# Fedomn/sqlrs

Hardware: AMD Instinct MI355X
Metric: Mrows/sec for filter->hash-join->group-by pipeline; achieved HBM GB/s vs peak (higher is better)
Workload: dtype int64 keys / f64 sum; 1 GPU; C5 filter(val>0.5) -> hash-join(fact x dim on int64 key) -> group-by(key) COUNT,SUM(f64); fact_rows=1000000000, dim_rows=10000000, groups=10000000, parallelism=single GPU

## Files before the change

sqlrs_amd/csrc/radix_part.hip:

```cpp
#include <cstdio>
#include <cstdlib>

#include "device_utils.hpp"
#include "radix_part.hpp"
#include "radix_part_kernels.hpp"

namespace sq {

namespace {

struct Level {
  std::vector<int64_t> seg_mat, seg_start;
  std::vector<uint32_t> seg_tiles, seg_tile_base;
  int64_t mat_entries = 0;
  uint32_t num_tiles = 0, nseg = 0;
  std::vector<uint8_t> blob;
  BufP dev, tiles;
  const int64_t *d_seg_start = nullptr, *d_seg_mat = nullptr;
  const uint32_t *d_seg_tiles = nullptr, *d_seg_tile_base = nullptr;
};

Level plan_level(const std::vector<int64_t> &seg_start, uint32_t digits, int RP_TILE) {
  Level L;
  L.seg_start = seg_start;
// ... 106 lines not shown
  };
  auto publish = [&](const Cols &c) {
    out->key = c.k; out->v0 = c.v0; out->v1 = c.v1; out->idx = c.idx; out->flags = c.fl; out->rec = c.rec;
  };
  struct SlimLaunch {
    SlimIn in;
    SlimOut out;
    uint32_t kshift, rbits;
    BufP total;
  };
  auto exec_level = [&](int level, uint32_t digits, const Level &L, const RpIn &rin, const RpOut &rout, int64_t sink,
                        BufP *offs_out, BufP premat = nullptr, SlimLaunch *slim = nullptr,
                        const std::function<void(const BufP &)> *before_scatter = nullptr) {
    const int64_t entries = std::max<int64_t>(L.mat_entries, 1);
    BufP mat = premat ? premat : ctx->alloc(4 * (size_t)entries);
    BufP offs = ctx->alloc(4 * (size_t)entries);
    BufP total = ctx->alloc(8);
    if (slim) slim->total = total;
    unsigned nt = L.num_tiles;
    const Tile *tp = (const Tile *)L.tiles->p;
    if (nt && !premat) {
      ProfScope ps(ctx, in.build_side ? "rp_hist_build" : "rp_hist");
#define SQ_RH1(R, PL) rp_hist_kernel<512, R, PL><<<dim3(nt), dim3(512), 0, ctx->stream>>>(rin.key, rin.key_validity, rin.flags, tp, P, p2_bits, level, digits, mat->as<uint32_t>(), kp)
#define SQ_RH(R) do { if (!rin.key_validity && !rin.flags) SQ_RH1(R, true); else SQ_RH1(R, false); } while (0)
      if (ROWS == 12) SQ_RH(12); else SQ_RH(8);
#undef SQ_RH
#undef SQ_RH1
      SQ_HIP(hipGetLastError());
    }
    BufP mat_dm = ctx->alloc(4 * (size_t)entries);
    BufP offs_tm = ctx->alloc(4 * (size_t)entries);
    const size_t tlds = (size_t)RP_TB * (digits + 1) * 4;
    const unsigned tblocks = (unsigned)ceil_div(nt, RP_TB);
    if (nt)
      rp_transpose_kernel<false><<<dim3(tblocks), dim3(256), tlds, ctx->stream>>>(
          mat->as<uint32_t>(), mat_dm->as<uint32_t>(), tp, nt, digits);
    exclusive_scan_u32(ctx, mat_dm->as<uint32_t>(), L.mat_entries, nullptr, offs->as<uint32_t>(),
                       total->as<uint64_t>());
    if (nt)
      rp_transpose_kernel<true><<<dim3(tblocks), dim3(256), tlds, ctx->stream>>>(
          offs->as<uint32_t>(), offs_tm->as<uint32_t>(), tp, nt, digits);
    SQ_HIP(hipGetLastError());
    if (before_scatter) (*before_scatter)(offs);
    if (nt) {
      ProfScope ps(ctx, in.build_side ? "rp_scatter_build" : "rp_scatter");
      uint32_t wgs = std::min<uint32_t>(nt, (uint32_t)ctx->num_cus);
      uint32_t tpw = (uint32_t)ceil_div(nt, wgs);
      wgs = (uint32_t)ceil_div(nt, tpw);
      dim3 g(wgs), b((unsigned)WG);
      const int mode = level == 1 ? (flags ? RP_L1_NULL : RP_L1) : (flags ? RP_LN_FLAG : RP_LN);
      if (slim) {
        const size_t slds = (size_t)RP_TILE * 13 + 1024 + (size_t)WG * 16 + 512 + 128;
        allow_big_lds(ctx, rp_scatter_slim_kernel);
        rp_scatter_slim_kernel<<<g, b, slds, ctx->stream>>>(slim->in, slim->out, tp, p2_bits, digits, offs_tm->as<uint32_t>(), nt, tpw, sink,
                                                           slim->kshift, slim->rbits);
        SQ_HIP(hipGetLastError());
        slim->total = total;
        *offs_out = offs;
        return;
      }
#define SQ_RP1(NV, R, M, PK)                                                                                  \
  do {                                                                                                        \
    constexpr bool can_rec = NV == 1 && PK;                                                                   \
    auto kfn = rp_scatter_kernel<NV, 512, R, M, PK>;                                                          \
    if (can_rec && rout.rec) kfn = rp_scatter_kernel<NV, 512, R, M, PK, can_rec>;                             \
    allow_big_lds(ctx, kfn);                                                                                  \
    kfn<<<g, b, lds, ctx->stream>>>(rin, rout, tp, P, p2_bits, level, digits, offs_tm->as<uint32_t>(), nt, tpw, \
                                    sink, kp);                                                                  \
  } while (0)
#define SQ_RP(NV, R)                                                                                          \
  do {                                                                                                        \
    if (mode == RP_L1) { if (pack) SQ_RP1(NV, R, RP_L1, true); else SQ_RP1(NV, R, RP_L1, false); }            \
    else if (mode == RP_L1_NULL) SQ_RP1(NV, R, RP_L1_NULL, false);                                            \
    else if (mode == RP_LN) { if (pack) SQ_RP1(NV, R, RP_LN, true); else SQ_RP1(NV, R, RP_LN, false); }       \
    else SQ_RP1(NV, R, RP_LN_FLAG, false);                                                                    \
  } while (0)
      if (nv == 2) SQ_RP(2, 8);
      else if (nv == 0) SQ_RP(0, 12); else SQ_RP(1, 12);
#undef SQ_RP1
#undef SQ_RP
      SQ_HIP(hipGetLastError());
    }
    *offs_out = offs;
  };

  auto run_level = [&](int level, uint32_t digits, const std::vector<int64_t> &seg_start, const RpIn &rin,
                       const RpOut &rout, BufP *offs_out, Level *L) {
    *L = plan_level(seg_start, digits, RP_TILE);
    L->tiles = ctx->alloc(sizeof(Tile) * (size_t)std::max<uint32_t>(L->num_tiles, 1));
    upload_level(ctx, *L);
    rp_make_tiles_kernel<<<dim3((unsigned)L->seg_tiles.size()), dim3(256), 0, ctx->stream>>>(
        L->d_seg_start, L->d_seg_mat, L->d_seg_tiles, L->d_seg_tile_base, RP_TILE, (Tile *)L->tiles->p);
    SQ_HIP(hipGetLastError());
    exec_level(level, digits, *L, rin, rout, n, offs_out);
  };

  auto bucket_starts = [&](const Level &L, const BufP &offs, uint32_t digits, int64_t rows,
                           std::vector<uint32_t> *host) -> BufP {
    uint32_t nseg = L.nseg;
    int64_t total = (int64_t)nseg * digits + 1;
    BufP bs = ctx->alloc(4 * (size_t)total);
    rp_bucket_starts_kernel<<<dim3((unsigned)ceil_div(total, 256)), dim3(256), 0, ctx->stream>>>(
        offs->as<uint32_t>(), L.d_seg_mat, L.d_seg_tiles, L.d_seg_start, digits, nseg, rows, bs->as<uint32_t>());
    SQ_HIP(hipGetLastError());
    if (4 * (size_t)total <= ctx->pinned_bytes) {
      const uint32_t *h = (const uint32_t *)ctx->fetch(bs->p, 4 * (size_t)total);
      host->assign(h, h + total);
// ... 79 lines not shown
        csl.log_b = log_b;
        csl.tile = (uint32_t)RP_TILE;
        csl.on = true;
      } else if (use_rec) cc.rec = ctx->alloc(16 * (size_t)pool_rows);
      else {
        cc.k = ctx->alloc(8 * (size_t)pool_rows);
        cc.v0 = nv >= 1 ? ctx->alloc(8 * (size_t)pool_rows) : nullptr;
      }
      ClaimOut co;
      co.key = cc.k ? cc.k->as<uint64_t>() : nullptr;
      co.v0 = cc.v0 ? cc.v0->as<uint64_t>() : nullptr;
      co.rec = cc.rec ? (u64x2 *)cc.rec->p : nullptr;
      co.cursor = cursor;
      co.rend = rend;
      co.kept = (unsigned long long *)cst;
      co.flag = (unsigned int *)(cst + 1);
      co.B = B;
      const int psrc = !in.filter.col ? -1 : ((nv >= 1 && (const void *)in.filter.col == in.vals[0]) ? 1 : 3);
      const size_t clds = (size_t)RP_TILE * 8 * (1 + nv) + (size_t)WG * (4 + 4 + 8 + 8);
      {
        ProfScope ps(ctx, in.filter.col ? "rp_claim_scatter_filter" : "rp_claim_scatter");
        const uint64_t *k = in.keys, *a0 = (const uint64_t *)in.vals[0];
        const int64_t sink = (int64_t)slots_max;
#define SQ_CL1(NV, PS, RC)                                                                                          \
  do {                                                                                                              \
    auto kfn = rp_claim_scatter_kernel<NV, 512, 12, PS, RC>;                                                        \
    allow_big_lds(ctx, kfn);                                                                                        \
    kfn<<<dim3(wgs), dim3(512), clds, ctx->stream>>>(k, a0, in.filter, n, co, P, tiles1c, tpw, sink, kp);           \
  } while (0)
#define SQ_CL(NV, RC)                                                                                               \
  do {                                                                                                              \
    if (psrc < 0) SQ_CL1(NV, -1, RC);                                                                               \
    else if (psrc == 1 && NV >= 1) SQ_CL1(NV, (NV >= 1 ? 1 : 3), RC);                                               \
    else SQ_CL1(NV, 3, RC);                                                                                         \
  } while (0)
        if (claim_slim) {
          SlimClaimOut so;
          so.rows = csl.rows;
          so.cursor = cursor;
          so.rend = rend;
          so.blk_bt = csl.blk_bt->as<uint32_t>();
          so.flag = co.flag;
          so.kept = co.kept;
          so.B = B;
          so.log_b = csl.log_b;
          const char *sd_e = hook("SQLRS_RP_SLIM_DELTA");
          so.max_delta = sd_e ? (uint32_t)std::max(1, std::min(std::atoi(sd_e), 127)) : 127u;
          const size_t slds = (size_t)RP_TILE * (8 + 4 + 2) + (size_t)WG * (4 + 4 + 8 + 8 + 4);
          const size_t slds768 = (size_t)RP_TILE * (8 + 4 + 2) + (size_t)768 * (4 + 4 + 8 + 8 + 4);
#define SQ_CS(W, R, PS, LDS)                                                                                        \
  do {                                                                                                              \
    auto kfn = rp_claim_scatter_slim_kernel<W, R, PS>;                                                              \
    allow_big_lds(ctx, kfn);                                                                                        \
    kfn<<<dim3(wgs), dim3(W), LDS, ctx->stream>>>(k, a0, in.filter, n, so, P, tiles1c, tpw, sink, kp);              \
  } while (0)
          if (psrc < 0) SQ_CS(768, 8, -1, slds768);
          else if (psrc == 1) SQ_CS(768, 8, 1, slds768);
          else SQ_CS(512, 12, 3, slds);
#undef SQ_CS
        } else if (nv == 0) SQ_CL(0, false);
        else if (use_rec) SQ_CL(1, true);
        else SQ_CL(1, false);
#undef SQ_CL
#undef SQ_CL1
        SQ_HIP(hipGetLastError());
      }
      const uint32_t *hp = (const uint32_t *)ctx->fetch(plan->p, plan_bytes);
      uint64_t hc[2];
      std::memcpy(hc, hp + plan_words, 16);
      if (!(uint32_t)hc[1]) {
        out->n = (int64_t)hc[0];
        out->P = P;
        publish(cc);
        if (claim_slim) out->slim = csl;
        out->bstart = plan;
        out->bstart_host.assign(hp, hp + P);
        out->bstart_host.push_back((uint32_t)slots_max);
        out->bend_host.assign(hp + 2 * (size_t)P, hp + 3 * (size_t)P);
        return true;
      }
    }
  }
  if (in.filter.col && p2_bits == 0) return false;

  static const int chunk_env = [] {
    const char *e = hook("SQLRS_RP_CHUNKED");
    return e ? std::atoi(e) : -1;
  }();
  const uint32_t tiles1 = (uint32_t)ceil_div(n, RP_TILE);
  uint32_t cwgs = std::min<uint32_t>(tiles1, (uint32_t)ctx->num_cus);
  if (const char *wg_e = hook("SQLRS_RP_CHUNK_WGS"))
    cwgs = std::max(1u, std::min<uint32_t>(cwgs, (uint32_t)std::atoi(wg_e)));
  const uint32_t ctpw = (uint32_t)ceil_div(tiles1, std::max(cwgs, 1u));
  cwgs = (uint32_t)ceil_div(tiles1, std::max(ctpw, 1u));
  const uint64_t spare_chunks = (uint64_t)cwgs * (d1 + 1);
  const uint64_t CAP = (uint64_t)RP_TILE;
  bool chunked = p2_bits != 0 && !flags && chunk_env != 0 && d1 <= (uint32_t)WG &&
                 (chunk_env == 1 || spare_chunks * CAP <= (uint64_t)n);
  if (in.filter.col && !chunked) return false;
  if (chunked) {
    const char *slim_e = hook("SQLRS_RP_SLIM");
    const bool slim_on = pack && kp.dense && nv == 1 && (size_t)P * 4 <= 24 * 1024 &&
                         kp.rbits + SLIM_LOCAL_BITS + 7 <= 32 && kp.rbits + p2_bits + SLIM_LOCAL_BITS <= 32 &&
                         !(slim_e && std::atoi(slim_e) == 0) && !(hook("SQLRS_RP_H2") && std::atoi(hook("SQLRS_RP_H2")) == 0);
    const char *sd_e = hook("SQLRS_RP_SLIM_DELTA");
    const uint32_t slim_delta = sd_e ? (uint32_t)std::max(1, std::min<int>(std::atoi(sd_e), (int)SLIM_RUNS - 1)) : SLIM_RUNS - 1;
    const uint64_t arena = (uint64_t)ctpw + d1 + 1 +
                           (slim_on ? (uint64_t)d1 * (uint64_t)ceil_div((int64_t)ctpw, (int64_t)slim_delta + 1) : 0);
    const uint64_t max_chunks = arena * cwgs;
    if (max_chunks * (CAP + RP_CHUNK_SKEW) + WG * (uint64_t)cwgs > 0xffffffffull) {
      if (in.filter.col) return false;
      chunked = false;
    }
    if (chunked && slim_on) {
      const size_t pool_rows = (size_t)max_chunks * (CAP + RP_CHUNK_SKEW) + (size_t)1024 * cwgs;
      const uint32_t digits2 = 1u << p2_bits;
      auto slim_alloc = [&](size_t rows, BufP &b0, BufP &b1) {
        SlimRowsView v;
        b0 = ctx->alloc(8 * rows);
        b1 = ctx->alloc(4 * rows);
        v.v = b0->as<uint64_t>();
        v.w = b1->as<uint32_t>();
        return v;
      };
      BufP cb0, cb1;
      BufP clen = ctx->alloc_zero(4 * (size_t)max_chunks);
      BufP cdig = ctx->alloc(4 * (size_t)max_chunks), cbase = ctx->alloc(4 * (size_t)max_chunks);
      BufP cstart = ctx->alloc(2 * (size_t)max_chunks * SLIM_RUNS);
      SQ_HIP(hipMemsetAsync(cstart->p, 0xff, 2 * (size_t)max_chunks * SLIM_RUNS, ctx->stream));
      BufP ctr = ctx->alloc_zero(8);
      BufP chist = ctx->alloc(4 * (size_t)max_chunks * digits2);
      SlimChunkOut so;
      so.rows = slim_alloc(pool_rows, cb0, cb1);
      so.chunk_len = clen->as<uint32_t>();
      so.chunk_dig = cdig->as<uint32_t>();
      so.chunk_base = cbase->as<uint32_t>();
      so.cstart = cstart->as<uint16_t>();
      so.counter = ctr->as<unsigned int>();
      so.max_chunks = (uint32_t)max_chunks;
      so.cap = (uint32_t)CAP;
      so.arena = (uint32_t)arena;
      so.hist = chist->as<uint32_t>();
      so.kshift = kp.rbits + p2_bits;
      so.max_delta = slim_delta;
      {
        const char *cc_e = hook("SQLRS_RP_CONC");
        so.conc_eighths = cc_e ? (uint32_t)std::max(1, std::min(std::atoi(cc_e), 9)) : 3u;
      }
      const int psrc = !in.filter.col ? -1 : ((const void *)in.filter.col == in.vals[0] ? 1 : 3);
      const size_t clds = (size_t)RP_TILE * 14 + (size_t)WG * (4 + 4 + 8 + 8 + 4 + 4) + (size_t)P * 4;
      {
        ProfScope ps(ctx, in.filter.col ? "rp_chunk_scatter_filter" : "rp_chunk_scatter");
        const int64_t sink = (int64_t)max_chunks * (CAP + RP_CHUNK_SKEW);
        const size_t clds768 = (size_t)RP_TILE * 14 + (size_t)768 * (4 + 4 + 8 + 8 + 4 + 4) + (size_t)P * 4;
#define SQ_SL(W, R, PS, LDS)                                                                                        \
  do {                                                                                                              \
    auto kfn = rp_chunk_scatter_slim_kernel<W, R, PS>;                                                              \
    allow_big_lds(ctx, kfn);                                                                                        \
    kfn<<<dim3(cwgs), dim3(W), LDS, ctx->stream>>>(in.keys, (const uint64_t *)in.vals[0], in.filter, n, so, P, p2_bits, d1, \
                                                   tiles1, ctpw, sink, kp);                                         \
  } while (0)
        if (psrc < 0) SQ_SL(768, 8, -1, clds768); else if (psrc == 1) SQ_SL(768, 8, 1, clds768); else SQ_SL(512, 12, 3, clds);
#undef SQ_SL
        SQ_HIP(hipGetLastError());
      }
      Level L2;
      L2.nseg = d1;
      const LevelLayout lay(d1);
      L2.dev = ctx->alloc(lay.total);
      bind_level(L2, lay);
      L2.tiles = ctx->alloc(sizeof(Tile) * (size_t)max_chunks);
      BufP totals = ctx->alloc(24);
      BufP tile_chunk = ctx->alloc(4 * (size_t)max_chunks);
      BufP plan = ctx->alloc(sizeof(ChunkPlan));
      SQ_HIP(hipMemsetAsync(plan->p, 0, sizeof(ChunkPlan), ctx->stream));
      const unsigned pblocks = (unsigned)std::min<uint64_t>(ceil_div((int64_t)max_chunks, 256 * 8), 128);
      rp_chunk_count_kernel<<<dim3(pblocks), dim3(256), 0, ctx->stream>>>(so.chunk_len, so.chunk_dig, so.counter, so.max_chunks,
                                                                        so.max_chunks, (uint32_t)RP_TILE, plan->as<ChunkPlan>());
      rp_chunk_prefix_kernel<<<dim3(1), dim3(64), 0, ctx->stream>>>(
          plan->as<ChunkPlan>(), so.counter, d1, digits2, (int64_t *)L2.d_seg_start, (int64_t *)L2.d_seg_mat,
          (uint32_t *)L2.d_seg_tiles, (uint32_t *)L2.d_seg_tile_base, totals->as<uint64_t>());
      rp_chunk_assign_kernel<<<dim3(pblocks), dim3(256), 0, ctx->stream>>>(
          so.chunk_len, so.chunk_dig, so.counter, so.max_chunks, so.max_chunks, digits2, (uint32_t)CAP, (uint32_t)RP_TILE,
          L2.d_seg_tiles, L2.d_seg_tile_base, plan->as<ChunkPlan>(), (Tile *)L2.tiles->p, tile_chunk->as<uint32_t>());
      SQ_HIP(hipGetLastError());
      const uint64_t *ht = (const uint64_t *)ctx->fetch(totals->p, 24);
      const uint64_t ntiles = ht[0], kept = ht[1], overflow = ht[2];
      if (overflow) return false;
      L2.num_tiles = (uint32_t)ntiles;
      L2.mat_entries = (int64_t)ntiles * digits2;
      out->n = (int64_t)kept;
      out->P = P;
      if (kept == 0) {
        out->bstart_host.assign((size_t)P + 1, 0u);
        out->bstart = nullptr;
        return true;
      }
      const size_t np = (size_t)kept + 1024;
      PartitionedRows::Slim &sl = out->slim;
      sl = PartitionedRows::Slim();
      sl.rows = slim_alloc(np, sl.buf0, sl.buf1);
      SlimLaunch sln;
      sln.in.rows = so.rows;
      sln.in.tile_chunk = tile_chunk->as<uint32_t>();
      sln.in.cstart = so.cstart;
      sln.out.rows = sl.rows;
      sln.kshift = so.kshift;
      sln.rbits = kp.rbits;
      BufP offs2;
      BufP premat = ctx->alloc(4 * (size_t)L2.mat_entries);
      rp_hist_from_chunks_kernel<<<dim3((unsigned)ceil_div(L2.mat_entries, 256)), dim3(256), 0, ctx->stream>>>(
          so.hist, tile_chunk->as<uint32_t>(), L2.mat_entries, digits2, premat->as<uint32_t>());
      SQ_HIP(hipGetLastError());
// ... 198 lines not shown
```

sqlrs_amd/csrc/radix_part_kernels.hpp:

```cpp
#pragma once
#include "device_utils.hpp"
#include "radix_part.hpp"

#ifdef RP_NT_STORES
#define RP_ST(ptr, val) __builtin_nontemporal_store((val), (ptr))
#else
#define RP_ST(ptr, val) (*(ptr) = (val))
#endif

namespace sq {


constexpr int vmcnt_imm(int n) { return (n & 0xF) | ((n >> 4) << 14) | 0x0F70; }

struct Tile {
  int64_t start;
  uint32_t len;
  uint32_t stride;
  int64_t mat;
};

__device__ __forceinline__ uint32_t xcd_tile(uint32_t b, uint32_t nb) {
  uint32_t q = nb >> 3, r = nb & 7, x = b & 7, i = b >> 3;
  return x * q + min(x, r) + i;
// ... 433 lines not shown
        if ((uint32_t)(j * RP_WG) < staged_len) store_row(j, staged_len);
        rank_row(j, len);
      }
#ifndef RP_PREFETCH_LATE
      __builtin_amdgcn_s_waitcnt(0x0F70);
#else
      rp_chunk_load<NV, RP_WG, RP_ROWS, PSRC>(key, v0, v1, flt.col, nstart, nlen, nxt);
      __builtin_amdgcn_s_waitcnt(vmcnt_imm(NLOADS < 63 ? NLOADS : 63));
#endif
      __syncthreads();
      scan_and_stage();
      staged_len = s_total;
      cur = nxt;
      len = nlen;
      cur_start = nstart;
    }
#pragma unroll
    for (int j = 0; j < RP_ROWS; j++)
      if ((uint32_t)(j * RP_WG) < staged_len) store_row(j, staged_len);
  }
  if (owner) {
    out.chunk_len[cur_id] = cfill;
    out.chunk_dig[cur_id] = threadIdx.x;
  }
  if (H2) {
    __syncthreads();
    close_id[threadIdx.x] = owner ? cur_id : 0xffffffffu;
    __syncthreads();
    flush_closed();
  }
}

constexpr uint32_t SLIM_RUNS = 128;
constexpr uint32_t SLIM_LOCAL_BITS = 13;
struct SlimChunkOut {
  SlimRowsView rows;
  uint32_t *chunk_len;
  uint32_t *chunk_dig;
  uint32_t *chunk_base;
  uint16_t *cstart;
  unsigned int *counter;
  uint32_t max_chunks, cap, arena;
  uint32_t *hist;
  uint32_t kshift;
  uint32_t max_delta;
  uint32_t conc_eighths;
};

template <int RP_ROWS> struct SlimCur {
  uint32_t off[RP_ROWS];
  uint64_t a0[RP_ROWS];
};

template <int RP_WG, int RP_ROWS, int PSRC>
__global__ __launch_bounds__(RP_WG, 1) void rp_chunk_scatter_slim_kernel(
    const uint64_t *__restrict__ key, const uint64_t *__restrict__ v0, RowFilter flt, int64_t n, SlimChunkOut out,
    uint32_t P, uint32_t p2_bits, uint32_t digits, uint32_t num_tiles, uint32_t tiles_per_wg, int64_t sink, KeyPack kp) {
  constexpr uint32_t RP_TILE = RP_WG * RP_ROWS;
  static_assert(RP_TILE <= (1u << SLIM_LOCAL_BITS), "row inside a tile must fit SLIM_LOCAL_BITS");
  extern __shared__ __attribute__((aligned(16))) unsigned char smem[];
  uint64_t *sv0 = (uint64_t *)smem;
  uint32_t *sw = (uint32_t *)(sv0 + RP_TILE);
  uint16_t *sdig = (uint16_t *)(sw + RP_TILE);
  uint32_t *cnt = (uint32_t *)(sdig + RP_TILE);
  uint32_t *split = cnt + RP_WG;
  int64_t *gb0 = (int64_t *)(split + RP_WG);
  int64_t *gb1 = gb0 + RP_WG;
  uint32_t *room_s = (uint32_t *)(gb1 + RP_WG);
  uint32_t *close_id = room_s + RP_WG;
  uint32_t *h2 = close_id + RP_WG;
  __shared__ uint32_t s_wsum[RP_WG / 64];
  __shared__ uint32_t s_total;
  __shared__ uint32_t s_next;
  const uint32_t d2n = 1u << p2_bits;
  const uint32_t inmask = (1u << out.kshift) - 1u;

  const uint32_t t0 = blockIdx.x * tiles_per_wg;
  const uint32_t t1 = min(num_tiles, t0 + tiles_per_wg);
  uint32_t cur_id = blockIdx.x * out.arena + min(threadIdx.x, digits - 1), cfill = 0, cbase = 0;
  bool opened = false;
  if (threadIdx.x == 0) s_next = digits;
  const bool owner = threadIdx.x < digits;
  room_s[threadIdx.x] = out.cap;
  for (uint32_t i = threadIdx.x; i < digits * d2n; i += RP_WG) h2[i] = 0;
  auto tile_start = [&](uint32_t t) { return (int64_t)t * RP_TILE; };
  auto tile_len = [&](uint32_t t) { return (uint32_t)min((int64_t)RP_TILE, n - (int64_t)t * RP_TILE); };

  ChunkRegs<1, RP_ROWS, PSRC> nxt;
  SlimCur<RP_ROWS> cur;
  uint32_t dr[RP_ROWS];
  uint32_t cur_tile = 0;
  auto take_rows = [&](uint32_t len, uint32_t nxt_tile, bool report) {
#pragma unroll
    for (int j = 0; j < RP_ROWS; j++) {
      bool keep = (uint32_t)(j * RP_WG) + threadIdx.x < len;
      if (PSRC == 1) keep = keep && row_passes(flt, nxt.a0[j]);
      if (PSRC == 3) keep = keep && row_passes(flt, nxt.pv[PSRC == 3 ? j : 0]);
      const uint64_t off = nxt.k[j] - kp.kmin;
      if (keep && off > kp.range) {
        if (kp.oob && report) key_out_of_range(kp, (uint32_t)((int64_t)nxt_tile * RP_TILE + (uint32_t)(j * RP_WG) + threadIdx.x));
        keep = false;
      }
      cur.off[j] = keep ? (uint32_t)off : 0xffffffffu;
      cur.a0[j] = nxt.a0[j];
    }
  };
  __shared__ uint32_t s_conc;
  uint32_t conc_digit = 0xffffffffu;
  uint32_t w_b0 = 0xffffffffu, w_base = 0;
  auto plan_wave = [&]() {
    w_b0 = 0xffffffffu;
    if (conc_digit == 0xffffffffu) return;
#pragma unroll
    for (int j = 0; j < RP_ROWS; j++) {
      const uint32_t bkt = cur.off[j] >> kp.rbits;
      const uint64_t m = __ballot(cur.off[j] != 0xffffffffu && (bkt >> p2_bits) == conc_digit);
      if (w_b0 == 0xffffffffu && m) w_b0 = (uint32_t)__builtin_amdgcn_readlane((int)bkt, __builtin_ctzll(m));
    }
    if (w_b0 == 0xffffffffu) return;
    uint32_t total = 0;
#pragma unroll
    for (int j = 0; j < RP_ROWS; j++)
      total += (uint32_t)__popcll(__ballot(cur.off[j] != 0xffffffffu && (cur.off[j] >> kp.rbits) == w_b0));
    if (total < 4u * RP_ROWS) {
      w_b0 = 0xffffffffu;
      return;
    }
    const uint32_t d0 = w_b0 >> p2_bits;
    uint32_t base = 0;
    if (lane_id() == 0) base = atomicAdd(&cnt[d0], total);
    w_base = (uint32_t)__builtin_amdgcn_readfirstlane((int)base);
    const uint32_t room = room_s[d0];
    const uint32_t nlo = room > w_base ? min(room - w_base, total) : 0u;
    if (lane_id() == 0) atomicAdd(&h2[w_b0], nlo + ((total - nlo) << 16));
  };
  auto rank_row = [&](int j) {
    dr[j] = 0xffffffffu;
    const bool in = cur.off[j] != 0xffffffffu;
    const uint32_t bkt = cur.off[j] >> kp.rbits;
    if (w_b0 != 0xffffffffu) {
      const bool peer = in && bkt == w_b0;
      const uint64_t same = __ballot(peer);
      if (peer) dr[j] = ((w_b0 >> p2_bits) << 16) | (w_base + (uint32_t)mbcnt(same));
      w_base += (uint32_t)__popcll(same);
      if (in && !peer) {
        const uint32_t d = bkt >> p2_bits;
        const uint32_t r = atomicAdd(&cnt[d], 1u);
        atomicAdd(&h2[bkt], r < room_s[d] ? 1u : 0x10000u);
        dr[j] = (d << 16) | r;
      }
      return;
    }
    if (in) {
      const uint32_t d = bkt >> p2_bits;
      const uint32_t r = atomicAdd(&cnt[d], 1u);
      atomicAdd(&h2[bkt], r < room_s[d] ? 1u : 0x10000u);
      dr[j] = (d << 16) | r;
    }
  };
  auto flush_closed = [&]() {
    for (uint32_t i = threadIdx.x; i < digits * d2n; i += RP_WG) {
      const uint32_t c = close_id[i >> p2_bits];
      if (c == 0xffffffffu) continue;
      const uint32_t v = h2[i];
      out.hist[(size_t)c * d2n + (i & (d2n - 1))] = v & 0xffffu;
      h2[i] = v >> 16;
    }
  };
  auto take_chunk = [&]() {
    const uint32_t o = atomicAdd(&s_next, 1u);
    if (o >= out.arena) out.counter[1] = 1;
    return blockIdx.x * out.arena + min(o, out.arena - 1);
  };
  auto scan_and_stage = [&]() {
    const uint32_t c = cnt[threadIdx.x];
    if (c * 8u >= (uint32_t)RP_TILE * out.conc_eighths) s_conc = threadIdx.x + 1;
    const uint32_t inc = wave_iscan_u32(c);
    if (lane_id() == 63) s_wsum[wave_id()] = inc;
    __syncthreads();
    conc_digit = s_conc - 1u;
    uint32_t wbase = 0, tot = 0;
    for (int w = 0; w < RP_WG / 64; w++) {
      if (w < wave_id()) wbase += s_wsum[w];
      tot += s_wsum[w];
    }
    const uint32_t ls = wbase + inc - c;
    if (threadIdx.x == 0) s_total = tot;
    const uint32_t room = min(c, out.cap - cfill);
    int64_t g0 = (int64_t)cur_id * (out.cap + RP_CHUNK_SKEW) + cfill, g1 = 0;
    uint32_t closing = 0xffffffffu;
    if (owner && c > 0) {
      if (!opened) {
        opened = true;
        cbase = cur_tile;
        out.chunk_base[cur_id] = cur_tile;
      }
      out.cstart[(size_t)cur_id * SLIM_RUNS + (cur_tile - cbase)] = (uint16_t)cfill;
    }
    if (owner && c > room) {
      out.chunk_len[cur_id] = out.cap;
      out.chunk_dig[cur_id] = threadIdx.x;
      closing = cur_id;
      cur_id = take_chunk();
      cfill = c - room;
      cbase = cur_tile;
      out.chunk_base[cur_id] = cur_tile;
      out.cstart[(size_t)cur_id * SLIM_RUNS] = 0;
      g1 = (int64_t)cur_id * (out.cap + RP_CHUNK_SKEW);
    } else {
      cfill += c;
      if (owner && opened && cur_tile + 1 - cbase > out.max_delta) {
        out.chunk_len[cur_id] = cfill;
        out.chunk_dig[cur_id] = threadIdx.x;
        closing = cur_id;
        cur_id = take_chunk();
        cfill = 0;
        opened = false;
      }
    }
    close_id[threadIdx.x] = closing;
    cnt[threadIdx.x] = ls;
    split[threadIdx.x] = ls + room;
    gb0[threadIdx.x] = g0 - (int64_t)ls;
    gb1[threadIdx.x] = g1 - (int64_t)(ls + room);
    room_s[threadIdx.x] = out.cap - cfill;
    __syncthreads();
    flush_closed();
#pragma unroll
    for (int j = 0; j < RP_ROWS; j++) {
      if (dr[j] == 0xffffffffu) continue;
      const uint32_t d = dr[j] >> 16;
      const uint32_t p = cnt[d] + (dr[j] & 0xffffu);
      const uint32_t local = (uint32_t)(j * RP_WG) + threadIdx.x;
      sv0[p] = cur.a0[j];
      sw[p] = (cur.off[j] & inmask) | (local << out.kshift);
      sdig[p] = (uint16_t)d;
    }
    __syncthreads();
  };
  auto store_row = [&](int j, uint32_t len) {
    const uint32_t p = j * RP_WG + threadIdx.x;
    const uint32_t d = min((uint32_t)sdig[p], (uint32_t)(RP_WG - 1));
    int64_t g = (p < split[d] ? gb0[d] : gb1[d]) + p;
    if (p >= len) g = sink + (int64_t)blockIdx.x * RP_WG + threadIdx.x;
    slim_store(out.rows, g, sw[p], sv0[p]);
  };

  if (t0 < t1) {
    uint32_t len = tile_len(t0);
    cur_tile = t0;
    rp_chunk_load<1, RP_WG, RP_ROWS, PSRC>(key, v0, nullptr, flt.col, tile_start(t0), len, nxt);
    __builtin_amdgcn_s_waitcnt(0x0F70);
    take_rows(len, t0, true);
    cnt[threadIdx.x] = 0;
    if (threadIdx.x == 0) s_conc = 0;
    __syncthreads();
    plan_wave();
#pragma unroll
    for (int j = 0; j < RP_ROWS; j++) rank_row(j);
    __syncthreads();
    scan_and_stage();
    uint32_t staged_len = s_total;
    uint32_t tcur = min(t0 + 1, t1 - 1);
    len = tile_len(tcur);
    cur_tile = tcur;
    rp_chunk_load<1, RP_WG, RP_ROWS, PSRC>(key, v0, nullptr, flt.col, tile_start(tcur), len, nxt);
    __builtin_amdgcn_s_waitcnt(0x0F70);
    take_rows(len, tcur, tcur != t0);
    for (uint32_t ti = t0 + 1; ti < t1; ti++) {
      const uint32_t tnext = min(ti + 1, t1 - 1);
      const uint32_t nlen = tile_len(tnext);
      rp_chunk_load<1, RP_WG, RP_ROWS, PSRC>(key, v0, nullptr, flt.col, tile_start(tnext), nlen, nxt);
      cnt[threadIdx.x] = 0;
      if (threadIdx.x == 0) s_conc = 0;
      __syncthreads();
      plan_wave();
#pragma unroll
      for (int j = 0; j < RP_ROWS; j++) {
        if ((uint32_t)(j * RP_WG) < staged_len) store_row(j, staged_len);
        rank_row(j);
      }
      __builtin_amdgcn_s_waitcnt(0x0F70);
      __syncthreads();
      scan_and_stage();
      staged_len = s_total;
      take_rows(nlen, tnext, tnext != ti);
      cur_tile = tnext;
    }
#pragma unroll
    for (int j = 0; j < RP_ROWS; j++)
      if ((uint32_t)(j * RP_WG) < staged_len) store_row(j, staged_len);
  }
  if (owner) {
    out.chunk_len[cur_id] = cfill;
    out.chunk_dig[cur_id] = threadIdx.x;
  }
  __syncthreads();
  close_id[threadIdx.x] = owner ? cur_id : 0xffffffffu;
  __syncthreads();
  flush_closed();
}

struct SlimIn {
  SlimRowsView rows;
  const uint32_t *tile_chunk;
  const uint16_t *cstart;
};
struct SlimOut {
  SlimRowsView rows;
};
template <int RP_ROWS> struct SlimRegs {
  uint64_t a0[RP_ROWS];
  uint32_t w[RP_ROWS];
  uint32_t goff;
  uint16_t cs0, cs1;
};
template <int RP_WG, int RP_ROWS>
__device__ __forceinline__ void rp_slim_load(const SlimIn &in, const Tile &t, uint32_t tile_index,
                                             const uint32_t *__restrict__ offs, uint32_t digits, SlimRegs<RP_ROWS> &r) {
#pragma unroll
  for (int j = 0; j < RP_ROWS; j++) {
    const int64_t row = t.start + min((uint32_t)(j * RP_WG) + threadIdx.x, t.len - 1);
    slim_load_nt(in.rows, row, r.w[j], r.a0[j]);
  }
  r.goff = offs[(int64_t)tile_index * digits + min(threadIdx.x, digits - 1)];
  const uint16_t *cs = in.cstart + (size_t)in.tile_chunk[tile_index] * SLIM_RUNS;
  r.cs0 = cs[lane_id()];
  r.cs1 = cs[64 + lane_id()];
}

__global__ __launch_bounds__(512, 1) void rp_scatter_slim_kernel(SlimIn in, SlimOut out, const Tile *__restrict__ tiles,
                                                                uint32_t p2_bits, uint32_t digits,
                                                                const uint32_t *__restrict__ offs, uint32_t num_tiles,
                                                                uint32_t tiles_per_wg, int64_t sink, uint32_t kshift,
                                                                uint32_t rbits) {
  constexpr int RP_WG = 512, RP_ROWS = 12, RP_TILE = RP_WG * RP_ROWS;
  static_assert(SLIM_RUNS == 128 && RP_TILE / 64 <= 128, "one mask word per 64 positions of a chunk");
  extern __shared__ __attribute__((aligned(16))) unsigned char smem[];
  uint64_t *sv0 = (uint64_t *)smem;
  unsigned long long *rmask = (unsigned long long *)(sv0 + RP_TILE);
  int64_t *gbase = (int64_t *)(rmask + 128);
  uint32_t *sw = (uint32_t *)(gbase + RP_WG);
  uint32_t *cnt = sw + RP_TILE;
  uint32_t *lstart = cnt + RP_WG;
  uint32_t *rpre = lstart + RP_WG;
  uint8_t *sdig = (uint8_t *)(rpre + 128);
  uint8_t *rdelta = sdig + RP_TILE;
  __shared__ uint32_t s_wsum[RP_WG / 64];
  __shared__ uint32_t s_psum;
  const uint32_t d2mask = (1u << p2_bits) - 1u, slotmask = (1u << rbits) - 1u;
  const uint64_t le_mask = (2ull << lane_id()) - 1ull;

  const uint32_t t0 = blockIdx.x * tiles_per_wg;
  const uint32_t t1 = min(num_tiles, t0 + tiles_per_wg);
  if (t0 >= t1) return;
  auto tile_of = [&](uint32_t slot) { return slot; };
  SlimRegs<RP_ROWS> cur, nxt;
  uint32_t dr[RP_ROWS];
  __shared__ uint32_t s_conc;
  bool conc_hint = false;
  auto rank_row = [&](int j, uint32_t len) {
    dr[j] = 0xffffffffu;
    const bool in = (uint32_t)(j * RP_WG) + threadIdx.x < len;
    const uint32_t d = (cur.w[j] >> rbits) & d2mask;
    if (conc_hint) {
      const uint64_t m = __ballot(in);
      if (m) {
        const int first = __builtin_ctzll(m);
        const uint32_t d0 = (uint32_t)__builtin_amdgcn_readlane((int)d, first);
        const bool peer = in && d == d0;
        const uint64_t same = __ballot(peer);
        if (__popcll(same) >= 8) {
          uint32_t base = 0;
          if ((int)lane_id() == first) base = atomicAdd(&cnt[d0], (uint32_t)__popcll(same));
          base = (uint32_t)__builtin_amdgcn_readlane((int)base, first);
          if (peer) dr[j] = (d0 << 16) | (base + (uint32_t)mbcnt(same));
          else if (in) dr[j] = (d << 16) | atomicAdd(&cnt[d], 1u);
          return;
        }
      }
    }
    if (in) dr[j] = (d << 16) | atomicAdd(&cnt[d], 1u);
  };
  auto build_runs = [&](uint32_t len) {
    if (wave_id() != 0) return;
    const bool f0 = cur.cs0 < len, f1 = cur.cs1 < len;
    const uint64_t b0 = __ballot(f0), b1 = __ballot(f1);
    const uint64_t lt = le_mask >> 1;
    if (f0) {
      rdelta[__popcll(b0 & lt)] = (uint8_t)lane_id();
      atomicOr(&rmask[cur.cs0 >> 6], 1ull << (cur.cs0 & 63));
    }
    if (f1) {
      rdelta[__popcll(b0) + __popcll(b1 & lt)] = (uint8_t)(64 + lane_id());
      atomicOr(&rmask[cur.cs1 >> 6], 1ull << (cur.cs1 & 63));
    }
  };
  auto scan_and_stage = [&](uint32_t tile_len) {
    uint32_t c = cnt[threadIdx.x];
    if (tile_len && c * 10u >= tile_len * 9u) s_conc = 1;
    uint32_t inc = wave_iscan_u32(c);
    if (lane_id() == 63) s_wsum[wave_id()] = inc;
    uint32_t pc = 0, pinc = 0;
    if (threadIdx.x < 128) {
      pc = (uint32_t)__popcll(rmask[threadIdx.x]);
      pinc = wave_iscan_u32(pc);
      if (threadIdx.x == 63) s_psum = pinc;
    }
    __syncthreads();
    conc_hint = s_conc != 0;
    uint32_t wbase = 0;
    for (int w = 0; w < wave_id(); w++) wbase += s_wsum[w];
    uint32_t ls = wbase + inc - c;
    lstart[threadIdx.x] = ls;
    gbase[threadIdx.x] = (int64_t)cur.goff - (int64_t)ls;
    if (threadIdx.x < 128) rpre[threadIdx.x] = pinc - pc + (threadIdx.x >= 64 ? s_psum : 0u);
    __syncthreads();
#pragma unroll
    for (int j = 0; j < RP_ROWS; j++) {
      if (dr[j] == 0xffffffffu) continue;
      const uint32_t p = lstart[dr[j] >> 16] + (dr[j] & 0xffffu);
      const uint32_t g = (uint32_t)(j * (RP_WG / 64)) + (uint32_t)wave_id();
      const uint32_t k = rpre[g] + (uint32_t)__popcll(rmask[g] & le_mask) - 1u;
      const uint32_t delta = rdelta[k & (SLIM_RUNS - 1)];
      const uint32_t w = cur.w[j];
      sv0[p] = cur.a0[j];
      sw[p] = (w & slotmask) | (((w >> kshift) & ((1u << SLIM_LOCAL_BITS) - 1u)) << rbits) | (delta << (rbits + SLIM_LOCAL_BITS));
      sdig[p] = (uint8_t)(dr[j] >> 16);
    }
    __syncthreads();
  };
  auto store_row = [&](int j, uint32_t len) {
    const uint32_t p = j * RP_WG + threadIdx.x;
    int64_t g = gbase[sdig[p] & d2mask] + p;
    if (p >= len) g = sink + threadIdx.x;
    slim_store(out.rows, g, sw[p], sv0[p]);
  };

  uint32_t tix = tile_of(t0);
  Tile t = tiles[tix];
  rp_slim_load<RP_WG, RP_ROWS>(in, t, tix, offs, digits, cur);
  __builtin_amdgcn_s_waitcnt(0x0F70);
  cnt[threadIdx.x] = 0;
  if (threadIdx.x < 128) rmask[threadIdx.x] = 0;
  if (threadIdx.x == 0) s_conc = 0;
  __syncthreads();
#pragma unroll
  for (int j = 0; j < RP_ROWS; j++) rank_row(j, t.len);
  build_runs(t.len);
  __syncthreads();
  scan_and_stage(t.len);
  uint32_t staged_len = t.len;
  tix = tile_of(min(t0 + 1, t1 - 1));
  t = tiles[tix];
  rp_slim_load<RP_WG, RP_ROWS>(in, t, tix, offs, digits, cur);
  __builtin_amdgcn_s_waitcnt(0x0F70);
  for (uint32_t ti = t0 + 1; ti < t1; ti++) {
    const uint32_t tnext = tile_of(min(ti + 1, t1 - 1));
    Tile tn = tiles[tnext];
    rp_slim_load<RP_WG, RP_ROWS>(in, tn, tnext, offs, digits, nxt);
    cnt[threadIdx.x] = 0;
    if (threadIdx.x < 128) rmask[threadIdx.x] = 0;
    if (threadIdx.x == 0) s_conc = 0;
    __syncthreads();
#pragma unroll
    for (int j = 0; j < RP_ROWS; j++) {
      store_row(j, staged_len);
      rank_row(j, t.len);
    }
    build_runs(t.len);
    __builtin_amdgcn_s_waitcnt(0x0F70);
    __syncthreads();
    scan_and_stage(t.len);
    staged_len = t.len;
    cur = nxt;
    t = tn;
  }
#pragma unroll
  for (int j = 0; j < RP_ROWS; j++) store_row(j, staged_len);
}

__global__ __launch_bounds__(256) void rp_slim_runs_kernel(const uint32_t *__restrict__ offs, int64_t entries,
                                                           const uint64_t *__restrict__ total, const int64_t *__restrict__ seg_mat,
                                                           const uint32_t *__restrict__ seg_tiles,
                                                           const uint32_t *__restrict__ seg_tile_base,
                                                           const uint32_t *__restrict__ tile_chunk,
                                                           const uint32_t *__restrict__ chunk_base, uint32_t digits,
                                                           uint32_t *__restrict__ nzstart, uint32_t *__restrict__ nzbt,
                                                           uint32_t *__restrict__ nzcount, uint32_t *__restrict__ bcol) {
  __shared__ uint32_t s_w[4];
  const uint32_t b = blockIdx.x, s = b / digits, d = b % digits;
  const uint32_t nt = seg_tiles[s];
  const int64_t col = seg_mat[s] + (int64_t)d * nt;
  uint32_t done = 0;
  for (uint32_t i0 = 0; i0 < nt; i0 += 256) {
    const uint32_t i = i0 + threadIdx.x;
    uint32_t start = 0, next = 0;
    if (i < nt) {
      start = offs[col + i];
      next = col + i + 1 < entries ? offs[col + i + 1] : (uint32_t)*total;
    }
    const bool f = i < nt && next > start;
    const uint64_t bal = __ballot(f);
    if (lane_id() == 0) s_w[wave_id()] = (uint32_t)__popcll(bal);
    __syncthreads();
    uint32_t before = done, all = 0;
    for (int w = 0; w < 4; w++) {
      if (w < wave_id()) before += s_w[w];
      all += s_w[w];
    }
    if (f) {
      const uint32_t k = before + (uint32_t)mbcnt(bal);
      nzstart[col + k] = start;
      nzbt[col + k] = chunk_base[tile_chunk[seg_tile_base[s] + i]];
    }
    done += all;
    __syncthreads();
  }
  if (threadIdx.x == 0) {
    nzcount[b] = done;
    bcol[b] = (uint32_t)col;
  }
}

struct ClaimOut {
  uint64_t *key, *v0;
  u64x2 *rec;
  uint32_t *cursor;
  const uint32_t *rend;
  unsigned int *flag;
  unsigned long long *kept;
  uint32_t B;
// ... 195 lines not shown
      const uint32_t tnext = min(ti + 1, t1 - 1);
      const uint32_t nlen = tile_len(tnext);
      const int64_t nstart = tile_start(tnext);
      rp_chunk_load<NV, RP_WG, RP_ROWS, PSRC>(key, v0, nullptr, flt.col, nstart, nlen, nxt);
      cnt[threadIdx.x] = 0;
      __syncthreads();
#pragma unroll
      for (int j = 0; j < RP_ROWS; j++) {
        if ((uint32_t)(j * RP_WG) < staged_len) store_row(j, staged_len);
        rank_row(j, len);
      }
      __builtin_amdgcn_s_waitcnt(0x0F70);
      __syncthreads();
      scan_and_stage();
      staged_len = s_total;
      cur = nxt;
      len = nlen;
      cur_start = nstart;
    }
#pragma unroll
    for (int j = 0; j < RP_ROWS; j++)
      if ((uint32_t)(j * RP_WG) < staged_len) store_row(j, staged_len);
  }
  if (owner && !dead) {
    for (uint32_t i = 0; i < room; i++) {
      if (REC) {
        u64x2 rec;
        rec.x = ~0ull;
        rec.y = 0;
        out.rec[pos + i] = rec;
      } else {
        out.key[pos + i] = ~0ull;
      }
    }
  }
  if (threadIdx.x == 0 && kept) atomicAdd(out.kept, kept);
}

struct SlimClaimOut {
  SlimRowsView rows;
  uint32_t *cursor;
  const uint32_t *rend;
  uint32_t *blk_bt;
  unsigned int *flag;
  unsigned long long *kept;
  uint32_t B, log_b;
  uint32_t max_delta;
};
constexpr uint32_t SLIM_SENTINEL = 0xffffffffu;

template <int RP_WG, int RP_ROWS, int PSRC>
__global__ __launch_bounds__(RP_WG, 1) void rp_claim_scatter_slim_kernel(
    const uint64_t *__restrict__ key, const uint64_t *__restrict__ v0, RowFilter flt, int64_t n, SlimClaimOut out, uint32_t P,
    uint32_t num_tiles, uint32_t tiles_per_wg, int64_t sink, KeyPack kp) {
  constexpr uint32_t RP_TILE = RP_WG * RP_ROWS;
  static_assert(RP_TILE < (1u << SLIM_LOCAL_BITS), "row 8191 of a tile is the sentinel");
  constexpr int64_t DEAD = -(1ll << 40);
  extern __shared__ __attribute__((aligned(16))) unsigned char smem[];
  uint64_t *sv0 = (uint64_t *)smem;
  uint32_t *sw = (uint32_t *)(sv0 + RP_TILE);
  uint16_t *sdig = (uint16_t *)(sw + RP_TILE);
  uint32_t *cnt = (uint32_t *)(sdig + RP_TILE);
  uint32_t *split = cnt + RP_WG;
  int64_t *gb0 = (int64_t *)(split + RP_WG);
  int64_t *gb1 = gb0 + RP_WG;
  uint32_t *dl0 = (uint32_t *)(gb1 + RP_WG);
  __shared__ uint32_t s_wsum[RP_WG / 64];
  __shared__ uint32_t s_total;

  const uint32_t t0 = blockIdx.x * tiles_per_wg;
  const uint32_t t1 = min(num_tiles, t0 + tiles_per_wg);
  const bool owner = threadIdx.x < P;
  uint32_t pos = 0, room = 0, bbase = 0;
  bool dead = false;
  const uint32_t my_end = owner ? out.rend[threadIdx.x] : 0u;
  const uint32_t Bm1 = out.B - 1;
  const uint32_t rbits = kp.rbits, smask = (1u << rbits) - 1u, dshift = rbits + SLIM_LOCAL_BITS;
  unsigned long long kept = 0;
  auto tile_start = [&](uint32_t t) { return (int64_t)t * RP_TILE; };
  auto tile_len = [&](uint32_t t) { return (uint32_t)min((int64_t)RP_TILE, n - (int64_t)t * RP_TILE); };

  ChunkRegs<1, RP_ROWS, PSRC> nxt;
  SlimCur<RP_ROWS> cur;
  uint32_t dr[RP_ROWS];
  uint32_t cur_tile = 0;
  auto take_rows = [&](uint32_t len, uint32_t nxt_tile, bool report, SlimCur<RP_ROWS> &cur) {
#pragma unroll
    for (int j = 0; j < RP_ROWS; j++) {
      bool keep = (uint32_t)(j * RP_WG) + threadIdx.x < len;
      if (PSRC == 1) keep = keep && row_passes(flt, nxt.a0[j]);
      if (PSRC == 3) keep = keep && row_passes(flt, nxt.pv[PSRC == 3 ? j : 0]);
      const uint64_t off = nxt.k[j] - kp.kmin;
      if (keep && off > kp.range) {
        if (kp.oob && report) key_out_of_range(kp, (uint32_t)((int64_t)nxt_tile * RP_TILE + (uint32_t)(j * RP_WG) + threadIdx.x));
        keep = false;
      }
      cur.off[j] = keep ? (uint32_t)off : 0xffffffffu;
      cur.a0[j] = nxt.a0[j];
    }
  };
  auto rank_row = [&](int j) {
    dr[j] = 0xffffffffu;
    if (cur.off[j] != 0xffffffffu) {
      const uint32_t d = min(cur.off[j] >> rbits, P - 1);
      dr[j] = (d << 16) | atomicAdd(&cnt[d], 1u);
    }
  };
// ... 16 lines not shown
    __syncthreads();
    uint32_t wbase = 0, tot = 0;
    for (int w = 0; w < RP_WG / 64; w++) {
      if (w < wave_id()) wbase += s_wsum[w];
      tot += s_wsum[w];
    }
    const uint32_t ls = wbase + inc - c;
    if (threadIdx.x == 0) {
      s_total = tot;
      kept += tot;
    }
    cnt[threadIdx.x] = ls;
    split[threadIdx.x] = ls + used;
    gb0[threadIdx.x] = (int64_t)pos - (int64_t)ls;
    dl0[threadIdx.x] = (cur_tile - bbase) << dshift;
    __syncthreads();
#pragma unroll
    for (int j = 0; j < RP_ROWS; j++) {
      if (dr[j] == 0xffffffffu) continue;
      const uint32_t d = dr[j] >> 16;
      const uint32_t p = cnt[d] + (dr[j] & 0xffffu);
      const uint32_t local = (uint32_t)(j * RP_WG) + threadIdx.x;
      sv0[p] = cur.a0[j];
      sw[p] = (cur.off[j] & smask) | (local << rbits) | (p < split[d] ? dl0[d] : 0u);
      sdig[p] = (uint16_t)d;
    }
    int64_t g1 = 0;
    if (claim) {
      if (!dead && (uint64_t)got + k > (uint64_t)my_end) {
        dead = true;
        *out.flag = 1u;
      }
      if (dead) {
        g1 = DEAD;
        pos = 0;
        room = 0;
      } else {
        g1 = (int64_t)got - (int64_t)(ls + used);
        pos = got + need;
        room = k - need;
        bbase = cur_tile;
        for (uint32_t b = got >> out.log_b, be = (got + k) >> out.log_b; b < be; b++) out.blk_bt[b] = cur_tile;
      }
    } else {
      pos += c;
      room -= c;
    }
    gb1[threadIdx.x] = g1;
    __syncthreads();
  };
  auto store_row = [&](int j, uint32_t len) {
    const uint32_t p = j * RP_WG + threadIdx.x;
    const uint32_t d = min((uint32_t)sdig[p], (uint32_t)(RP_WG - 1));
    int64_t g = (p < split[d] ? gb0[d] : gb1[d]) + p;
    if (p >= len || g < 0) g = sink + (int64_t)blockIdx.x * RP_WG + threadIdx.x;
    slim_store(out.rows, g, sw[p], sv0[p]);
  };

  if (t0 < t1) {
    uint32_t len = tile_len(t0);
    cur_tile = t0;
    rp_chunk_load<1, RP_WG, RP_ROWS, PSRC>(key, v0, nullptr, flt.col, tile_start(t0), len, nxt);
    __builtin_amdgcn_s_waitcnt(0x0F70);
    take_rows(len, t0, true, cur);
    cnt[threadIdx.x] = 0;
    __syncthreads();
#pragma unroll
    for (int j = 0; j < RP_ROWS; j++) rank_row(j);
    __syncthreads();
    scan_and_stage();
    uint32_t staged_len = s_total;
    uint32_t tcur = min(t0 + 1, t1 - 1);
    len = tile_len(tcur);
    cur_tile = tcur;
    rp_chunk_load<1, RP_WG, RP_ROWS, PSRC>(key, v0, nullptr, flt.col, tile_start(tcur), len, nxt);
    __builtin_amdgcn_s_waitcnt(0x0F70);
    take_rows(len, tcur, tcur != t0, cur);
    for (uint32_t ti = t0 + 1; ti < t1; ti++) {
      const uint32_t tnext = min(ti + 1, t1 - 1);
      const uint32_t nlen = tile_len(tnext);
      rp_chunk_load<1, RP_WG, RP_ROWS, PSRC>(key, v0, nullptr, flt.col, tile_start(tnext), nlen, nxt);
      cnt[threadIdx.x] = 0;
      __syncthreads();
#pragma unroll
      for (int j = 0; j < RP_ROWS; j++) {
        if ((uint32_t)(j * RP_WG) < staged_len) store_row(j, staged_len);
        rank_row(j);
      }
      __builtin_amdgcn_s_waitcnt(0x0F70);
      __syncthreads();
      scan_and_stage();
      staged_len = s_total;
      take_rows(nlen, tnext, tnext != ti, cur);
      cur_tile = tnext;
    }
#pragma unroll
    for (int j = 0; j < RP_ROWS; j++)
      if ((uint32_t)(j * RP_WG) < staged_len) store_row(j, staged_len);
  }
  if (owner && !dead) fill_sentinels(pos, room);
  if (threadIdx.x == 0 && kept) atomicAdd(out.kept, kept);
}

struct ChunkPlan {
  uint32_t seg_tiles[512];
  uint32_t cursor[512];
  unsigned long long seg_rows[512];
};
__global__ __launch_bounds__(256) void rp_chunk_count_kernel(const uint32_t *__restrict__ chunk_len,
// ... 120 lines not shown
```

Before: 94930 Mrows/s.

## Stage chunk run starts in LDS and drop sink-row scatter stores

Replaces the sink-row trick for padding or dead rows in three slim scatter kernels with predicated stores, and skips whole store rows past the staged length. This removes wasted global writes and the extra pool rows reserved for the sink. The chunk scatter kernel also gains an LDS-resident run-start table per digit, used when LDS allows. It is flushed to global memory only when a chunk closes, replacing scattered 16-bit global writes per tile. The cost is extra LDS use and more flush logic, plus predication that can cause divergence.

New measurement: 92340 Mrows/s. -2.7%, worse.

```diff
diff --git a/sqlrs_amd/csrc/radix_part.hip b/sqlrs_amd/csrc/radix_part.hip
--- a/sqlrs_amd/csrc/radix_part.hip
+++ b/sqlrs_amd/csrc/radix_part.hip
@@ -182,7 +182,7 @@
       if (slim) {
         const size_t slds = (size_t)RP_TILE * 13 + 1024 + (size_t)WG * 16 + 512 + 128;
         allow_big_lds(ctx, rp_scatter_slim_kernel);
-        rp_scatter_slim_kernel<<<g, b, slds, ctx->stream>>>(slim->in, slim->out, tp, p2_bits, digits, offs_tm->as<uint32_t>(), nt, tpw, sink,
+        rp_scatter_slim_kernel<<<g, b, slds, ctx->stream>>>(slim->in, slim->out, tp, p2_bits, digits, offs_tm->as<uint32_t>(), nt, tpw,
                                                            slim->kshift, slim->rbits);
         SQ_HIP(hipGetLastError());
         slim->total = total;
@@ -368,7 +368,7 @@
   do {                                                                                                              \
     auto kfn = rp_claim_scatter_slim_kernel<W, R, PS>;                                                              \
     allow_big_lds(ctx, kfn);                                                                                        \
-    kfn<<<dim3(wgs), dim3(W), LDS, ctx->stream>>>(k, a0, in.filter, n, so, P, tiles1c, tpw, sink, kp);              \
+    kfn<<<dim3(wgs), dim3(W), LDS, ctx->stream>>>(k, a0, in.filter, n, so, P, tiles1c, tpw, kp);                    \
   } while (0)
           if (psrc < 0) SQ_CS(768, 8, -1, slds768);
           else if (psrc == 1) SQ_CS(768, 8, 1, slds768);
@@ -429,7 +429,7 @@
       chunked = false;
     }
     if (chunked && slim_on) {
-      const size_t pool_rows = (size_t)max_chunks * (CAP + RP_CHUNK_SKEW) + (size_t)1024 * cwgs;
+      const size_t pool_rows = (size_t)max_chunks * (CAP + RP_CHUNK_SKEW);
       const uint32_t digits2 = 1u << p2_bits;
       auto slim_alloc = [&](size_t rows, BufP &b0, BufP &b1) {
         SlimRowsView v;
@@ -467,14 +467,15 @@
       const size_t clds = (size_t)RP_TILE * 14 + (size_t)WG * (4 + 4 + 8 + 8 + 4 + 4) + (size_t)P * 4;
       {
         ProfScope ps(ctx, in.filter.col ? "rp_chunk_scatter_filter" : "rp_chunk_scatter");
-        const int64_t sink = (int64_t)max_chunks * (CAP + RP_CHUNK_SKEW);
         const size_t clds768 = (size_t)RP_TILE * 14 + (size_t)768 * (4 + 4 + 8 + 8 + 4 + 4) + (size_t)P * 4;
+        const size_t runs_lds = (size_t)d1 * SLIM_RUNS * 2;
 #define SQ_SL(W, R, PS, LDS)                                                                                        \
   do {                                                                                                              \
-    auto kfn = rp_chunk_scatter_slim_kernel<W, R, PS>;                                                              \
+    const bool lruns = (LDS) + runs_lds <= (size_t)149 * 1024;                                                      \
+    auto kfn = lruns ? rp_chunk_scatter_slim_kernel<W, R, PS, true> : rp_chunk_scatter_slim_kernel<W, R, PS, false>; \
     allow_big_lds(ctx, kfn);                                                                                        \
-    kfn<<<dim3(cwgs), dim3(W), LDS, ctx->stream>>>(in.keys, (const uint64_t *)in.vals[0], in.filter, n, so, P, p2_bits, d1, \
-                                                   tiles1, ctpw, sink, kp);                                         \
+    kfn<<<dim3(cwgs), dim3(W), (LDS) + (lruns ? runs_lds : 0), ctx->stream>>>(                                      \
+        in.keys, (const uint64_t *)in.vals[0], in.filter, n, so, P, p2_bits, d1, tiles1, ctpw, kp);                \
   } while (0)
         if (psrc < 0) SQ_SL(768, 8, -1, clds768); else if (psrc == 1) SQ_SL(768, 8, 1, clds768); else SQ_SL(512, 12, 3, clds);
 #undef SQ_SL
diff --git a/sqlrs_amd/csrc/radix_part_kernels.hpp b/sqlrs_amd/csrc/radix_part_kernels.hpp
--- a/sqlrs_amd/csrc/radix_part_kernels.hpp
+++ b/sqlrs_amd/csrc/radix_part_kernels.hpp
@@ -509,10 +509,10 @@
   uint64_t a0[RP_ROWS];
 };
 
-template <int RP_WG, int RP_ROWS, int PSRC>
+template <int RP_WG, int RP_ROWS, int PSRC, bool LRUNS>
 __global__ __launch_bounds__(RP_WG, 1) void rp_chunk_scatter_slim_kernel(
     const uint64_t *__restrict__ key, const uint64_t *__restrict__ v0, RowFilter flt, int64_t n, SlimChunkOut out,
-    uint32_t P, uint32_t p2_bits, uint32_t digits, uint32_t num_tiles, uint32_t tiles_per_wg, int64_t sink, KeyPack kp) {
+    uint32_t P, uint32_t p2_bits, uint32_t digits, uint32_t num_tiles, uint32_t tiles_per_wg, KeyPack kp) {
   constexpr uint32_t RP_TILE = RP_WG * RP_ROWS;
   static_assert(RP_TILE <= (1u << SLIM_LOCAL_BITS), "row inside a tile must fit SLIM_LOCAL_BITS");
   extern __shared__ __attribute__((aligned(16))) unsigned char smem[];
@@ -526,9 +526,13 @@
   uint32_t *room_s = (uint32_t *)(gb1 + RP_WG);
   uint32_t *close_id = room_s + RP_WG;
   uint32_t *h2 = close_id + RP_WG;
+  uint16_t *runs = (uint16_t *)(h2 + P);
+  constexpr uint32_t RESPILL = 0x80000000u;
   __shared__ uint32_t s_wsum[RP_WG / 64];
   __shared__ uint32_t s_total;
   __shared__ uint32_t s_next;
+  __shared__ uint32_t s_nclose;
+  __shared__ uint16_t s_clist[RP_WG];
   const uint32_t d2n = 1u << p2_bits;
   const uint32_t inmask = (1u << out.kshift) - 1u;
 
@@ -540,6 +544,8 @@
   const bool owner = threadIdx.x < digits;
   room_s[threadIdx.x] = out.cap;
   for (uint32_t i = threadIdx.x; i < digits * d2n; i += RP_WG) h2[i] = 0;
+  if (LRUNS)
+    for (uint32_t i = threadIdx.x; i < digits * (SLIM_RUNS / 2); i += RP_WG) ((uint32_t *)runs)[i] = 0xffffffffu;
   auto tile_start = [&](uint32_t t) { return (int64_t)t * RP_TILE; };
   auto tile_len = [&](uint32_t t) { return (uint32_t)min((int64_t)RP_TILE, n - (int64_t)t * RP_TILE); };
 
@@ -617,11 +623,22 @@
   };
   auto flush_closed = [&]() {
     for (uint32_t i = threadIdx.x; i < digits * d2n; i += RP_WG) {
-      const uint32_t c = close_id[i >> p2_bits];
+      uint32_t c = close_id[i >> p2_bits];
       if (c == 0xffffffffu) continue;
+      if (LRUNS) c &= ~RESPILL;
       const uint32_t v = h2[i];
       out.hist[(size_t)c * d2n + (i & (d2n - 1))] = v & 0xffffu;
       h2[i] = v >> 16;
+    }
+    if (LRUNS) {
+      const uint32_t nc = s_nclose;
+      for (uint32_t i = threadIdx.x; i < nc * (SLIM_RUNS / 2); i += RP_WG) {
+        const uint32_t d = s_clist[i / (SLIM_RUNS / 2)], e = i % (SLIM_RUNS / 2);
+        const uint32_t c = close_id[d];
+        uint32_t *row = (uint32_t *)runs + d * (SLIM_RUNS / 2);
+        ((uint32_t *)out.cstart)[(size_t)(c & ~RESPILL) * (SLIM_RUNS / 2) + e] = row[e];
+        row[e] = (e == 0 && (c & RESPILL)) ? 0xffff0000u : 0xffffffffu;
+      }
     }
   };
   auto take_chunk = [&]() {
@@ -652,7 +669,8 @@
         cbase = cur_tile;
         out.chunk_base[cur_id] = cur_tile;
       }
-      out.cstart[(size_t)cur_id * SLIM_RUNS + (cur_tile - cbase)] = (uint16_t)cfill;
+      if (LRUNS) runs[threadIdx.x * SLIM_RUNS + (cur_tile - cbase)] = (uint16_t)cfill;
+      else out.cstart[(size_t)cur_id * SLIM_RUNS + (cur_tile - cbase)] = (uint16_t)cfill;
     }
     if (owner && c > room) {
       out.chunk_len[cur_id] = out.cap;
@@ -662,7 +680,8 @@
       cfill = c - room;
       cbase = cur_tile;
       out.chunk_base[cur_id] = cur_tile;
-      out.cstart[(size_t)cur_id * SLIM_RUNS] = 0;
+      if (LRUNS) closing |= RESPILL;
+      else out.cstart[(size_t)cur_id * SLIM_RUNS] = 0;
       g1 = (int64_t)cur_id * (out.cap + RP_CHUNK_SKEW);
     } else {
       cfill += c;
@@ -676,6 +695,7 @@
       }
     }
     close_id[threadIdx.x] = closing;
+    if (LRUNS && closing != 0xffffffffu) s_clist[atomicAdd(&s_nclose, 1u)] = (uint16_t)threadIdx.x;
     cnt[threadIdx.x] = ls;
     split[threadIdx.x] = ls + room;
     gb0[threadIdx.x] = g0 - (int64_t)ls;
@@ -698,9 +718,8 @@
   auto store_row = [&](int j, uint32_t len) {
     const uint32_t p = j * RP_WG + threadIdx.x;
     const uint32_t d = min((uint32_t)sdig[p], (uint32_t)(RP_WG - 1));
-    int64_t g = (p < split[d] ? gb0[d] : gb1[d]) + p;
-    if (p >= len) g = sink + (int64_t)blockIdx.x * RP_WG + threadIdx.x;
-    slim_store(out.rows, g, sw[p], sv0[p]);
+    const int64_t g = (p < split[d] ? gb0[d] : gb1[d]) + p;
+    if (p < len) slim_store(out.rows, g, sw[p], sv0[p]);
   };
 
   if (t0 < t1) {
@@ -711,6 +730,7 @@
     take_rows(len, t0, true);
     cnt[threadIdx.x] = 0;
     if (threadIdx.x == 0) s_conc = 0;
+    if (LRUNS && threadIdx.x == 0) s_nclose = 0;
     __syncthreads();
     plan_wave();
 #pragma unroll
@@ -730,6 +750,7 @@
       rp_chunk_load<1, RP_WG, RP_ROWS, PSRC>(key, v0, nullptr, flt.col, tile_start(tnext), nlen, nxt);
       cnt[threadIdx.x] = 0;
       if (threadIdx.x == 0) s_conc = 0;
+      if (LRUNS && threadIdx.x == 0) s_nclose = 0;
       __syncthreads();
       plan_wave();
 #pragma unroll
@@ -754,6 +775,8 @@
   }
   __syncthreads();
   close_id[threadIdx.x] = owner ? cur_id : 0xffffffffu;
+  if (LRUNS && owner) s_clist[threadIdx.x] = (uint16_t)threadIdx.x;
+  if (LRUNS && threadIdx.x == 0) s_nclose = digits;
   __syncthreads();
   flush_closed();
 }
@@ -789,8 +812,7 @@
 __global__ __launch_bounds__(512, 1) void rp_scatter_slim_kernel(SlimIn in, SlimOut out, const Tile *__restrict__ tiles,
                                                                 uint32_t p2_bits, uint32_t digits,
                                                                 const uint32_t *__restrict__ offs, uint32_t num_tiles,
-                                                                uint32_t tiles_per_wg, int64_t sink, uint32_t kshift,
-                                                                uint32_t rbits) {
+                                                                uint32_t tiles_per_wg, uint32_t kshift, uint32_t rbits) {
   constexpr int RP_WG = 512, RP_ROWS = 12, RP_TILE = RP_WG * RP_ROWS;
   static_assert(SLIM_RUNS == 128 && RP_TILE / 64 <= 128, "one mask word per 64 positions of a chunk");
   extern __shared__ __attribute__((aligned(16))) unsigned char smem[];
@@ -889,9 +911,8 @@
   };
   auto store_row = [&](int j, uint32_t len) {
     const uint32_t p = j * RP_WG + threadIdx.x;
-    int64_t g = gbase[sdig[p] & d2mask] + p;
-    if (p >= len) g = sink + threadIdx.x;
-    slim_store(out.rows, g, sw[p], sv0[p]);
+    const int64_t g = gbase[sdig[p] & d2mask] + p;
+    if (p < len) slim_store(out.rows, g, sw[p], sv0[p]);
   };
 
   uint32_t tix = tile_of(t0);
@@ -922,7 +943,7 @@
     __syncthreads();
 #pragma unroll
     for (int j = 0; j < RP_ROWS; j++) {
-      store_row(j, staged_len);
+      if ((uint32_t)(j * RP_WG) < staged_len) store_row(j, staged_len);
       rank_row(j, t.len);
     }
     build_runs(t.len);
@@ -934,7 +955,8 @@
     t = tn;
   }
 #pragma unroll
-  for (int j = 0; j < RP_ROWS; j++) store_row(j, staged_len);
+  for (int j = 0; j < RP_ROWS; j++)
+    if ((uint32_t)(j * RP_WG) < staged_len) store_row(j, staged_len);
 }
 
 __global__ __launch_bounds__(256) void rp_slim_runs_kernel(const uint32_t *__restrict__ offs, int64_t entries,
@@ -1236,7 +1258,7 @@
 template <int RP_WG, int RP_ROWS, int PSRC>
 __global__ __launch_bounds__(RP_WG, 1) void rp_claim_scatter_slim_kernel(
     const uint64_t *__restrict__ key, const uint64_t *__restrict__ v0, RowFilter flt, int64_t n, SlimClaimOut out, uint32_t P,
-    uint32_t num_tiles, uint32_t tiles_per_wg, int64_t sink, KeyPack kp) {
+    uint32_t num_tiles, uint32_t tiles_per_wg, KeyPack kp) {
   constexpr uint32_t RP_TILE = RP_WG * RP_ROWS;
   static_assert(RP_TILE < (1u << SLIM_LOCAL_BITS), "row 8191 of a tile is the sentinel");
   constexpr int64_t DEAD = -(1ll << 40);
@@ -1359,9 +1381,8 @@
   auto store_row = [&](int j, uint32_t len) {
     const uint32_t p = j * RP_WG + threadIdx.x;
     const uint32_t d = min((uint32_t)sdig[p], (uint32_t)(RP_WG - 1));
-    int64_t g = (p < split[d] ? gb0[d] : gb1[d]) + p;
-    if (p >= len || g < 0) g = sink + (int64_t)blockIdx.x * RP_WG + threadIdx.x;
-    slim_store(out.rows, g, sw[p], sv0[p]);
+    const int64_t g = (p < split[d] ? gb0[d] : gb1[d]) + p;
+    if (p < len && g >= 0) slim_store(out.rows, g, sw[p], sv0[p]);
   };
 
   if (t0 < t1) {
```
